# techshoww/RoMa

Measured on AMD Instinct MI355X. Metric: image-pairs/sec at 560->864, higher is better.
Workload: dtype fp16; 1 GPU; roma_outdoor 560->864 full coarse-to-fine symmetric match (BASELINE configs[1]; configs[2] = --pairs 8 --gpus 8); launch=eager launches, coarse_res=560, upsample_res=864, parallelism=single GPU

## Files before the change

include/roma_hip.h:

```cpp
#ifndef ROMA_HIP_H
#define ROMA_HIP_H

#include <stdint.h>

#ifdef __cplusplus
extern "C" {
#endif

#define ROMA_ABI_VERSION 5

enum { ROMA_F32 = 0, ROMA_F16 = 1, ROMA_BF16 = 2 };
enum { ROMA_NCHW = 0, ROMA_NHWC = 1 };
enum { ROMA_LC_AUTO = 0, ROMA_LC_TILE8X4 = 1, ROMA_LC_TILE8X8 = 2, ROMA_LC_ROWS8 = 3 };
enum { ROMA_E_ARG = -1, ROMA_E_DTYPE = -2, ROMA_E_SHAPE = -3, ROMA_E_ALIGN = -4, ROMA_E_UNSUPPORTED = -5 };

int roma_abi_version(void);
const char* roma_last_error(void);

int roma_local_corr(const void* f0, const void* f1, const float* flow, void* out,
                    int B, int C, int H, int W, int r, int dtype,
                    int layout, int f0_pitch, int f1_pitch, int out_layout, int out_pitch, int f1_batch_shift, int variant,
                    void* stream);

int roma_warp_bilinear(const void* src, const float* flow, void* dst,
                       int B, int C, int Hs, int Ws, int H, int W, int dtype,
                       int layout, int src_pitch, int dst_layout, int dst_pitch, int src_batch_shift, void* stream);

int roma_disp_emb(const float* flow, const float* weight, const float* bias, void* dst,
                  int B, int E, int H, int W, float gain, int dtype, int dst_layout, int dst_pitch, void* stream);

int roma_interp_bilinear(const float* x, float* y, int N, int Hi, int Wi, int Ho, int Wo, void* stream);

int roma_interp_bilinear_pair(const float* x0, float* y0, int N0, const float* x1, float* y1, int N1, int Hi, int Wi, int Ho, int Wo,
                              void* stream);

int roma_refiner_assemble(const void* src, const float* flow, const float* weight, const float* bias, void* buf, int B, int C, int E,
                          int D, int pitch, int Hs, int Ws, int H, int W, int src_pitch, int src_batch_shift, float gain, int dtype,
                          void* stream);

int roma_flow_update(float* flow, float* cert, const float* cert_in, const float* delta,
                     int B, int H, int W, float sx, float sy, void* stream);

int roma_cls_to_flow_refine(const void* logits, float* flow_out, float* cert_out,
                            int B, int C, int HW, long stride_b, long stride_c, long stride_p,
                            int dtype, void* stream);

int roma_cos_kernel(const void* x, const void* y, float* K, int B, int N, int M, int D, int dtype, int x_pitch, int y_pitch,
                    int y_batch_shift, float T, float eps, float diag_add, void* stream);

int roma_chol_diag_block(float* A, int lda, long strideA, float* W, int ldw, long strideW, int nb, int B, int* info,
                         int info_base, void* stream);

int roma_chol_step(float* A, int lda, long strideA, int n, int ncols, int j, int nb, const float* W, int ldw, long strideW, float* R,
                   int ldr, long strideR, float* Wn, int ldwn, long strideWn, int* info, int info_base, int B, void* stream);

int roma_chol_subst_step(int dir, const float* W, int ldw, long strideW, const float* R, long strideRb, long strideRs, int ldr, float* T,
                         long strideTb, long strideTs, int ldt, int t_in_panel, float* X, int ldx, long strideX, int n, int m, int nb,
                         int s, int B, void* stream);

int roma_attention_fwd(const void* q, const void* k, const void* v, void* o, int B, int H, int Nq, int Nk, int head_dim, long q_sb,
                       long q_sn, long q_sh, long k_sb, long k_sn, long k_sh, long v_sb, long v_sn, long v_sh, long o_sb, long o_sn,
                       long o_sh, float scale, int dtype, void* stream);

int roma_match_finalize(const float* flow, const float* cert, const float* cert16, float* warp, float* certainty,
                        int P, int H, int W, int H16, int W16, int symmetric, void* stream);

int roma_kde_density(const float* x, float* density, int N, int down, float std, int half_mode, void* stream);

int roma_race_keys(const float* p, const long* counter, float* keys, long N, float thresh, unsigned seed, unsigned stage,
                   void* stream);

long roma_race_select_workspace(int P, long N, int k);
int roma_race_select(const float* p, const long* counter, const long* seeds, int P, long N, int k, float thresh, unsigned stage,
                     long* sel_key, long* sel_idx, void* workspace, long workspace_bytes, void* stream);

int roma_kde_density_batch(const float* x, const long* index, float* density, int P, long N, int n, int down, float std,
                           int half_mode, void* stream);

int roma_nn_argmin(const float* q, const float* r, int* idx, int NQ, int NR, void* stream);

int roma_resample_u8(const void* in, void* out, int H, int W, int C, int out_size, int axis, const int* bounds,
                     const int* coef, int ksize, void* stream);
int roma_normalize_u8(const void* in, float* out, int H, int W, const float* mean3, const float* std3, void* stream);

int roma_bias_relu_nchw(void* x, const void* bias, int B, int C, int HW, int dtype, void* stream);

int roma_bias_relu_pool2_nchw(void* x, const void* bias, void* pooled, int B, int C, int H, int W, int dtype, void* stream);

int roma_bias_relu_nhwc(void* x, const void* bias, long npix, int C, int dtype, void* stream);
int roma_bias_relu_pool2_nhwc(void* x, const void* bias, void* pooled, int B, int C, int H, int W, int dtype, void* stream);

int roma_maxpool2_nhwc(const void* x, void* pooled, int B, int C, int H, int W, int dtype, void* stream);

int roma_conv3x3_bias_relu(const void* x, const void* w, const void* bias, void* y, int B, int Cin, int Cout, int H, int W, int dtype,
                           int x_pitch, int y_pitch, int instance, void* stream);
int roma_conv3x3_bias_relu_instances(int index, char* name, int cap);

int roma_dwconv5x5_bn_relu(const void* x, const float* w, const float* scale, const float* shift, void* y,
                           int B, int C, int H, int W, int dtype, int x_pitch, int y_pitch, void* stream);

int roma_refiner_block(const void* x, const void* w25, const float* scale, const float* shift, const void* wt,
                       const float* bias, void* y, int B, int C, int H, int W, int kpad, int dtype, int x_pitch, int y_pitch,
                       void* stream);

int roma_refiner_wide_pack(const void* wt, void* wp, int D);
int roma_refiner_wide_taps(const void* w25, void* w25p, int D);
int roma_refiner_block_wide(const void* x, const void* w25p, const float* scale, const float* shift, const void* wp,
                            const float* bias, void* y, int B, int H, int W, int D, int x_pitch, int y_pitch, int dtype,
                            void* stream);

int roma_pointwise_mfma(const void* x, const void* wt, const float* bias, void* y, long M, int C, int kpad, int dtype,
                        int x_pitch, int y_pitch, void* stream);

int roma_refiner_block_mid(const void* x, const float* w25, const float* scale, const float* shift, const void* wt,
                           const float* bias, void* y, int B, int C, int H, int W, int dtype, int x_pitch, int y_pitch,
                           void* stream);

int roma_refiner_head(const void* x, const float* wo, const float* bo, float* flow, const float* cert_in, float* cert_out,
                      float* delta_out, int B, int H, int W, int C, int pitch, int dtype, float sx, float sy, void* stream);

int roma_pointwise_small(const void* x, const float* wt, const float* bias, void* y, long M, int C, int dtype,
                         int x_pitch, int y_pitch, void* stream);

int roma_project_skinny(const void* x, const void* wt, const float* bias, void* y, long M, int K, int N, int dtype, int x_pitch,
                        int y_pitch, void* stream);

int roma_add_layernorm(void* x, int x_dtype, long x_stride, const void* y, int y_dtype, long y_stride, const float* ls,
                       const float* gamma, const float* beta, void* out, int out_dtype, long out_stride, long rows, int C,
                       float eps, void* stream);

int roma_tiny_corr_posembed(const float* f0, const float* f1, float* out, int B, int C,
// ... 114 lines not shown
```

roma_amd/_lib.py:

```python
from __future__ import annotations

import ctypes
import os
from ctypes import c_char_p, c_float, c_int, c_long, c_void_p

_HERE = os.path.dirname(os.path.abspath(__file__))
LIB_PATH = os.path.join(_HERE, "csrc", "libroma_hip.so")

ROMA_F32, ROMA_F16, ROMA_BF16 = 0, 1, 2
ROMA_NCHW, ROMA_NHWC = 0, 1
LC_VARIANTS = {"auto": 0, "tile8x4": 1, "tile8x8": 2, "rows8": 3}
ABI_VERSION = 5
SCORE_MSAC, SCORE_MAGSAC = 0, 1
ROMA_E_ARG, ROMA_E_DTYPE, ROMA_E_SHAPE, ROMA_E_ALIGN, ROMA_E_UNSUPPORTED = -1, -2, -3, -4, -5

SIGNATURES = {
    "roma_abi_version": [],
    "roma_last_error": [],
    "roma_local_corr": [c_void_p, c_void_p, c_void_p, c_void_p, c_int, c_int, c_int, c_int, c_int, c_int,
                        c_int, c_int, c_int, c_int, c_int, c_int, c_int, c_void_p],
    "roma_warp_bilinear": [c_void_p, c_void_p, c_void_p, c_int, c_int, c_int, c_int, c_int, c_int, c_int,
                           c_int, c_int, c_int, c_int, c_int, c_void_p],
    "roma_disp_emb": [c_void_p, c_void_p, c_void_p, c_void_p, c_int, c_int, c_int, c_int, c_float, c_int, c_int, c_int, c_void_p],
    "roma_interp_bilinear": [c_void_p, c_void_p, c_int, c_int, c_int, c_int, c_int, c_void_p],
    "roma_interp_bilinear_pair": [c_void_p, c_void_p, c_int, c_void_p, c_void_p, c_int, c_int, c_int, c_int, c_int, c_void_p],
    "roma_refiner_assemble": [c_void_p, c_void_p, c_void_p, c_void_p, c_void_p, c_int, c_int, c_int, c_int, c_int, c_int, c_int, c_int,
                              c_int, c_int, c_int, c_float, c_int, c_void_p],
    "roma_project_skinny": [c_void_p, c_void_p, c_void_p, c_void_p, c_long, c_int, c_int, c_int, c_int, c_int, c_void_p],
    "roma_flow_update": [c_void_p, c_void_p, c_void_p, c_void_p, c_int, c_int, c_int, c_float, c_float, c_void_p],
    "roma_cls_to_flow_refine": [c_void_p, c_void_p, c_void_p, c_int, c_int, c_int, c_long, c_long, c_long, c_int, c_void_p],
    "roma_cos_kernel": [c_void_p, c_void_p, c_void_p, c_int, c_int, c_int, c_int, c_int, c_int, c_int, c_int, c_float, c_float,
                        c_float, c_void_p],
    "roma_add_layernorm": [c_void_p, c_int, c_long, c_void_p, c_int, c_long, c_void_p, c_void_p, c_void_p, c_void_p, c_int, c_long,
                           c_long, c_int, c_float, c_void_p],
    "roma_attention_fwd": [c_void_p, c_void_p, c_void_p, c_void_p, c_int, c_int, c_int, c_int, c_int] + [c_long] * 12 + [c_float, c_int, c_void_p],
    "roma_chol_diag_block": [c_void_p, c_int, c_long, c_void_p, c_int, c_long, c_int, c_int, c_void_p, c_int, c_void_p],
    "roma_chol_step": [c_void_p, c_int, c_long, c_int, c_int, c_int, c_int, c_void_p, c_int, c_long, c_void_p, c_int, c_long,
                       c_void_p, c_int, c_long, c_void_p, c_int, c_int, c_void_p],
    "roma_chol_subst_step": [c_int, c_void_p, c_int, c_long, c_void_p, c_long, c_long, c_int, c_void_p, c_long, c_long, c_int, c_int,
                             c_void_p, c_int, c_long, c_int, c_int, c_int, c_int, c_int, c_void_p],
    "roma_match_finalize": [c_void_p, c_void_p, c_void_p, c_void_p, c_void_p, c_int, c_int, c_int, c_int, c_int, c_int, c_void_p],
    "roma_kde_density": [c_void_p, c_void_p, c_int, c_int, c_float, c_int, c_void_p],
    "roma_nn_argmin": [c_void_p, c_void_p, c_void_p, c_int, c_int, c_void_p],
    "roma_race_keys": [c_void_p, c_void_p, c_void_p, c_long, c_float, ctypes.c_uint, ctypes.c_uint, c_void_p],
    "roma_race_select_workspace": [c_int, c_long, c_int],
    "roma_race_select": [c_void_p, c_void_p, c_void_p, c_int, c_long, c_int, c_float, ctypes.c_uint, c_void_p, c_void_p, c_void_p, c_long,
                         c_void_p],
    "roma_kde_density_batch": [c_void_p, c_void_p, c_void_p, c_int, c_long, c_int, c_int, c_float, c_int, c_void_p],
    "roma_dwconv5x5_bn_relu": [c_void_p, c_void_p, c_void_p, c_void_p, c_void_p, c_int, c_int, c_int, c_int, c_int, c_int, c_int, c_void_p],
    "roma_resample_u8": [c_void_p, c_void_p, c_int, c_int, c_int, c_int, c_int, c_void_p, c_void_p, c_int, c_void_p],
    "roma_normalize_u8": [c_void_p, c_void_p, c_int, c_int, c_void_p, c_void_p, c_void_p],
    "roma_bias_relu_nchw": [c_void_p, c_void_p, c_int, c_int, c_int, c_int, c_void_p],
    "roma_bias_relu_pool2_nchw": [c_void_p, c_void_p, c_void_p, c_int, c_int, c_int, c_int, c_int, c_void_p],
    "roma_bias_relu_nhwc": [c_void_p, c_void_p, c_long, c_int, c_int, c_void_p],
    "roma_bias_relu_pool2_nhwc": [c_void_p, c_void_p, c_void_p, c_int, c_int, c_int, c_int, c_int, c_void_p],
    "roma_maxpool2_nhwc": [c_void_p, c_void_p, c_int, c_int, c_int, c_int, c_int, c_void_p],
    "roma_conv3x3_bias_relu": [c_void_p, c_void_p, c_void_p, c_void_p, c_int, c_int, c_int, c_int, c_int, c_int, c_int, c_int, c_int, c_void_p],
    "roma_conv3x3_bias_relu_instances": [c_int, c_char_p, c_int],
    "roma_pointwise_mfma": [c_void_p, c_void_p, c_void_p, c_void_p, c_long, c_int, c_int, c_int, c_int, c_int, c_void_p],
    "roma_refiner_block": [c_void_p, c_void_p, c_void_p, c_void_p, c_void_p, c_void_p, c_void_p, c_int, c_int, c_int, c_int, c_int, c_int,
                           c_int, c_int, c_void_p],
    "roma_refiner_block_mid": [c_void_p, c_void_p, c_void_p, c_void_p, c_void_p, c_void_p, c_void_p, c_int, c_int, c_int, c_int, c_int, c_int,
                               c_int, c_void_p],
    "roma_refiner_wide_pack": [c_void_p, c_void_p, c_int],
    "roma_refiner_wide_taps": [c_void_p, c_void_p, c_int],
    "roma_jpeg_info": [c_void_p, c_long, c_void_p],
    "roma_jpeg_entropy_decode": [c_void_p, c_long, c_void_p, c_void_p],
    "roma_jpeg_reconstruct": [c_void_p, c_void_p, c_void_p, c_void_p, c_void_p, c_void_p],
    "roma_refiner_block_wide": [c_void_p, c_void_p, c_void_p, c_void_p, c_void_p, c_void_p, c_void_p, c_int, c_int, c_int, c_int, c_int, c_int,
                                c_int, c_void_p],
    "roma_refiner_head": [c_void_p, c_void_p, c_void_p, c_void_p, c_void_p, c_void_p, c_void_p, c_int, c_int, c_int, c_int, c_int, c_int,
                          c_float, c_float, c_void_p],
    "roma_pointwise_small": [c_void_p, c_void_p, c_void_p, c_void_p, c_long, c_int, c_int, c_int, c_int, c_void_p],
    "roma_tiny_corr_posembed": [c_void_p, c_void_p, c_void_p, c_int, c_int, c_int, c_int, c_int, c_int, c_int, c_void_p],
    "roma_ransac_workspace": [c_int, c_int, c_int, c_int, c_void_p],
    "roma_ransac_hypotheses": [c_int, c_void_p, c_void_p, c_int, c_int, c_int, c_float, ctypes.c_uint, c_int, c_void_p, c_long, c_void_p],
    "roma_ransac_select": [c_int, c_void_p, c_void_p, c_int, c_int, c_int, c_float, c_int, c_void_p, c_long, c_void_p, c_void_p,
                           c_void_p],
    "roma_ransac_hypotheses_ex": [c_int, c_void_p, c_void_p, c_int, c_int, c_int, c_float, c_int, ctypes.c_uint, c_int, c_void_p, c_long,
                                  c_void_p],
    "roma_ransac_select_ex": [c_int, c_void_p, c_void_p, c_int, c_int, c_int, c_float, c_int, c_int, c_void_p, c_long, c_void_p, c_void_p,
                              c_void_p],
    "roma_magsac_table": [c_void_p, c_void_p],
    "roma_essential_workspace": [c_int, c_int, c_int, c_void_p],
    "roma_essential_hypotheses": [c_void_p, c_void_p, c_void_p, c_void_p, c_int, c_int, c_int, c_float, ctypes.c_uint, c_int, c_void_p,
                                  c_long, c_void_p],
    "roma_essential_select": [c_void_p, c_void_p, c_void_p, c_void_p, c_int, c_int, c_int, c_float, c_int, c_void_p, c_long, c_void_p,
                              c_void_p, c_void_p],
    "roma_essential_hypotheses_ex": [c_void_p, c_void_p, c_void_p, c_void_p, c_int, c_int, c_int, c_float, c_int, ctypes.c_uint, c_int,
                                     c_void_p, c_long, c_void_p],
    "roma_essential_select_ex": [c_void_p, c_void_p, c_void_p, c_void_p, c_int, c_int, c_int, c_float, c_int, c_int, c_void_p, c_long,
                                 c_void_p, c_void_p, c_void_p],
    "roma_recover_pose": [c_void_p, c_void_p, c_void_p, c_void_p, c_void_p, c_void_p, c_int, c_int, c_void_p, c_void_p, c_void_p,
                          c_void_p, c_void_p],
    "roma_refine_pose": [c_void_p, c_void_p, c_void_p, c_void_p, c_void_p, c_void_p, c_void_p, c_int, c_int, ctypes.c_double, c_int,
                         c_void_p, c_void_p, c_void_p, c_void_p, c_void_p, c_void_p, c_void_p],
    "roma_refine_fundamental": [c_void_p, c_void_p, c_void_p, c_void_p, c_int, c_int, ctypes.c_double, c_int, c_void_p, c_void_p, c_void_p,
                                c_void_p, c_void_p, c_void_p],
    "roma_refine_homography": [c_void_p, c_void_p, c_void_p, c_void_p, c_int, c_int, ctypes.c_double, c_int, c_void_p, c_void_p, c_void_p,
                               c_void_p, c_void_p, c_void_p],
    "roma_triangulate": [c_void_p, c_void_p, c_void_p, c_void_p, c_void_p, c_void_p, c_void_p, c_int, c_int, c_int, c_float, c_float,
                         c_void_p, c_void_p, c_void_p, c_void_p, c_void_p, c_void_p, c_void_p],
    "roma_triangulate_nview": [c_void_p, c_void_p, c_void_p, c_long, c_void_p, c_void_p, c_void_p, c_int, c_int, c_int, c_long, c_long,
                               c_float, c_int, c_int, c_int, c_float, c_float, c_void_p, c_void_p, c_void_p, c_void_p, c_void_p, c_void_p,
                               c_void_p],
    "roma_tracks_workspace": [c_int, c_void_p, c_int, c_void_p],
    "roma_build_tracks": [c_void_p, c_void_p, c_void_p, c_void_p, c_void_p, c_int, c_int, c_int, c_int, c_float, c_int, c_int, c_void_p,
                          c_void_p, c_void_p, c_void_p, c_void_p, c_void_p, c_void_p, c_long, c_void_p],
    "roma_warp_kpts": [c_void_p, c_int, c_void_p, c_void_p, c_void_p, c_void_p, c_void_p, c_int, c_int, c_int, c_int, c_int, c_int, c_int,
                       ctypes.c_double, c_void_p, c_void_p, c_void_p, c_void_p],
    "roma_dense_match_metrics": [c_void_p, c_long, c_void_p, c_void_p, c_void_p, c_void_p, c_void_p, c_int, c_int, c_int, c_int, c_int, c_int,
                                 c_int, c_int, ctypes.c_double, c_void_p, c_long, c_void_p, c_void_p, c_void_p, c_void_p, c_void_p],
    "roma_absolute_pose_workspace": [c_int, c_int, c_int, c_void_p],
    "roma_absolute_pose_hypotheses": [c_void_p, c_void_p, c_void_p, c_int, c_int, c_int, c_float, c_int, ctypes.c_uint, c_int, c_void_p,
                                      c_long, c_void_p],
# ... 63 lines not shown
```

roma_amd/csrc/cos_kernel.hip:

```cpp
#include "common.h"

namespace roma {
namespace {

typedef float f32x16 __attribute__((ext_vector_type(16)));
constexpr int BT = 64, KT = 16, LD = KT + 1;

template <typename T> __device__ __forceinline__ float4_t ld4(const T* p) {
  if constexpr (sizeof(T) == 4) {
    return *reinterpret_cast<const float4_t*>(p);
  } else {
    typedef T v4 __attribute__((ext_vector_type(4)));
    const v4 h = *reinterpret_cast<const v4*>(p);
    return float4_t{(float)h[0], (float)h[1], (float)h[2], (float)h[3]};
  }
}

template <typename T>
__global__ __launch_bounds__(256) void cos_kernel_mfma(const T* __restrict__ x, const T* __restrict__ y, float* __restrict__ K,
                                                       int N, int M, int D, int x_pitch, int y_pitch, int y_shift, float invT,
                                                       float eps, float diag_add) {
  __shared__ float sA[BT * LD], sB[BT * LD];
  __shared__ double sN[2 * BT];
  const int tid = threadIdx.x, lane = tid & 63, wave = tid >> 6;
  const int wr = wave >> 1, wc = wave & 1;
  const int b = blockIdx.z, n0 = blockIdx.y * BT, m0 = blockIdx.x * BT;
  const T* xb = x + (size_t)b * N * x_pitch;
  const T* yb = y + (size_t)((b + y_shift) % (int)gridDim.z) * M * y_pitch;
  f32x16 acc;
  double accd[16];
#pragma unroll
  for (int i = 0; i < 16; ++i) { acc[i] = 0.f; accd[i] = 0.0; }
  double nrm = 0.0;
  const int lr = tid >> 2, lc = (tid & 3) * 4;
  for (int k0 = 0; k0 < D; k0 += KT) {
    float4_t va{0, 0, 0, 0}, vb{0, 0, 0, 0};
    if (n0 + lr < N) va = ld4<T>(xb + (size_t)(n0 + lr) * x_pitch + k0 + lc);
    if (m0 + lr < M) vb = ld4<T>(yb + (size_t)(m0 + lr) * y_pitch + k0 + lc);
    __syncthreads();
#pragma unroll
    for (int i = 0; i < 4; ++i) {
      sA[lr * LD + lc + i] = va[i];
      sB[lr * LD + lc + i] = vb[i];
    }
    __syncthreads();
    if (tid < 2 * BT) {
      const float* r = (tid < BT ? sA : sB) + (tid & (BT - 1)) * LD;
#pragma unroll
      for (int i = 0; i < KT; ++i) nrm = __builtin_fma((double)r[i], (double)r[i], nrm);
    }
    const float* pa = sA + (wr * 32 + (lane & 31)) * LD + (lane >> 5);
    const float* pb = sB + (wc * 32 + (lane & 31)) * LD + (lane >> 5);
#pragma unroll
    for (int kk = 0; kk < KT; kk += 2) acc = __builtin_amdgcn_mfma_f32_32x32x2f32(pa[kk], pb[kk], acc, 0, 0, 0);
    if (((k0 / KT) & 3) == 3 || k0 + KT >= D) {
#pragma unroll
      for (int i = 0; i < 16; ++i) { accd[i] += (double)acc[i]; acc[i] = 0.f; }
    }
  }
  if (tid < 2 * BT) sN[tid] = sqrt(nrm);
  __syncthreads();
  const int col = lane & 31;
  const int m = m0 + wc * 32 + col;
  const double ny = sN[BT + wc * 32 + col];
#pragma unroll
  for (int r = 0; r < 16; ++r) {
    const int row = (r & 3) + 8 * (r >> 2) + 4 * (lane >> 5);
    const int n = n0 + wr * 32 + row;
    if (n < N && m < M) {
      const double c = accd[r] / (sN[wr * 32 + row] * ny + (double)eps);
      float v = (float)exp((c - 1.0) * (double)invT);
      if (n == m) v += diag_add;
      K[((size_t)b * N + n) * M + m] = v;
    }
  }
}

}
}

using namespace roma;

extern "C" int roma_cos_kernel(const void* x, const void* y, float* K, int B, int N, int M, int D, int dtype, int x_pitch,
                               int y_pitch, int y_batch_shift, float T, float eps, float diag_add, void* stream) {
  ROMA_REQUIRE(x && y && K, ROMA_E_ARG, "roma_cos_kernel: null pointer");
  ROMA_REQUIRE(B > 0 && N > 0 && M > 0 && D > 0, ROMA_E_SHAPE, "roma_cos_kernel: bad shape");
  ROMA_REQUIRE(D % KT == 0, ROMA_E_SHAPE, "roma_cos_kernel: D=%d must be a multiple of %d", D, KT);
  ROMA_REQUIRE(x_pitch >= D && y_pitch >= D, ROMA_E_SHAPE, "roma_cos_kernel: row pitch smaller than D");
  ROMA_REQUIRE(dtype >= ROMA_F32 && dtype <= ROMA_BF16, ROMA_E_DTYPE, "roma_cos_kernel: unknown dtype %d", dtype);
  const int e16 = dtype == ROMA_F32 ? 4 : 8;
  ROMA_REQUIRE(aligned16(x) && aligned16(y) && x_pitch % e16 == 0 && y_pitch % e16 == 0, ROMA_E_ALIGN,
               "roma_cos_kernel: x and y must be 16-byte aligned with row pitches that keep every row 16-byte aligned");
  ROMA_REQUIRE(y_batch_shift >= 0 && y_batch_shift < B, ROMA_E_ARG, "roma_cos_kernel: y_batch_shift %d outside [0, B)", y_batch_shift);
  ROMA_REQUIRE(T > 0.f, ROMA_E_ARG, "roma_cos_kernel: temperature must be positive");
  dim3 grid((M + BT - 1) / BT, (N + BT - 1) / BT, B);
  hipStream_t s = static_cast<hipStream_t>(stream);
#define ROMA_COS(TT)                                                                                                         \
  hipLaunchKernelGGL((cos_kernel_mfma<TT>), grid, dim3(256), 0, s, (const TT*)x, (const TT*)y, K, N, M, D, x_pitch, y_pitch, \
                     y_batch_shift, 1.f / T, eps, diag_add)
  if (dtype == ROMA_F32) ROMA_COS(float); else if (dtype == ROMA_F16) ROMA_COS(half_t); else ROMA_COS(bf16_t);
#undef ROMA_COS
  ROMA_CHECK_LAUNCH();
}
```

roma_amd/matcher.py:

```python
from __future__ import annotations

import math
import os
from collections import namedtuple
from typing import Dict, Optional
from warnings import warn

import numpy as np
import torch
import torch.nn as nn
import torch.nn.functional as F

from . import ops
from .transformer import Block, TransformerDecoder

IMAGENET_MEAN = (0.485, 0.456, 0.406)
IMAGENET_STD = (0.229, 0.224, 0.225)


def pixel_grid(b, h, w, device):
    ys = torch.linspace(-1 + 1 / h, 1 - 1 / h, h, device=device)
    xs = torch.linspace(-1 + 1 / w, 1 - 1 / w, w, device=device)
    return torch.stack((xs[None, :].expand(h, w), ys[:, None].expand(h, w)), dim=0)[None].expand(b, 2, h, w).contiguous()

# ... 168 lines not shown
                if impl == "split_mfma":
                    cur = ops.pointwise_mfma(rows, blk.wt_out_in, blk.bias, Dp)
                elif impl == "split_small":
                    cur = ops.pointwise_small(rows, blk.wt_in_out, blk.bias)
                else:
                    cur = torch.addmm(blk.bias, rows, blk.wt_in_out)
                cur = cur.view(B, h, w, Dp)
        return cur, P

    @torch.no_grad()
    def forward(self, x, y, flow, scale_factor=1, logits=None, dtype=None):
        flow = flow.float().contiguous()
        cur, P = self._body(x, y, flow, scale_factor, dtype or self.amp_dtype)
        B, h, w, Dp = cur.shape
        out = torch.addmm(P.bo, cur.reshape(B * h * w, Dp).float(), P.wo)
        out = out.view(B, h, w, self.out_dim).permute(0, 3, 1, 2).contiguous()
        return out[:, :-1], out[:, -1:]

    @torch.no_grad()
    def forward_update(self, x, y, flow, certainty, scale_factor, sx, sy, dtype=None, buf=None, batch_shift=0):
        cur, P = self._body(x, y, flow, scale_factor, dtype or self.amp_dtype, buf=buf, batch_shift=batch_shift)
        return ops.refiner_head(cur, P.wo, P.bo, flow, certainty, sx, sy)


class CosKernel(nn.Module):
    def __init__(self, T=0.2, learn_temperature=False):
        super().__init__()
        self.T = T

    def __call__(self, x, y, eps=1e-6):
        return ops.cos_kernel(x, y, T=self.T, eps=eps)


class GP(nn.Module):

    def __init__(self, gp_dim=512, T=0.2, sigma_noise=0.1, kernel=None, **_):
        super().__init__()
        self.K = CosKernel(T=T)
        self.sigma_noise = sigma_noise
        self.pos_conv = nn.Conv2d(2, gp_dim, 1, 1)
        self.dim = gp_dim
        self._basis = {}

    def basis(self, b, h, w, device):
        key = (h, w, device, _params_version(self.pos_conv))
        f = self._basis.get(key)
        if f is None:
            g = pixel_grid(1, h, w, device)
            f = torch.cos(8 * math.pi * F.conv2d(g, self.pos_conv.weight.float(), self.pos_conv.bias.float()))
            f = f.flatten(2).transpose(1, 2).contiguous()
            self._basis = {key: f}
        return f.expand(b, -1, -1)

    @torch.no_grad()
    def forward(self, x, y, **kwargs):
        b, c, h1, w1 = x.shape
        _, _, h2, w2 = y.shape
        xs = x.float().flatten(2).transpose(1, 2).contiguous()
        ys = y.float().flatten(2).transpose(1, 2).contiguous()
        K_yy = ops.cos_kernel(ys, ys, T=self.K.T, diag_add=self.sigma_noise)
        K_xy = ops.cos_kernel(xs, ys, T=self.K.T)
        mu = self.posterior_product(K_xy, ops.spd_solve(K_yy, self.basis(1, h2, w2, x.device)))
        return mu.transpose(1, 2).reshape(b, self.dim, h1, w1)

    def posterior_rows(self, xs, ys, h2, w2, fp64=False, batch_shift=0, out=None, check="now"):
        B, n = xs.shape[0], xs.shape[1]
        s = batch_shift % B
        basis = self.basis(1, h2, w2, xs.device)
        if fp64:
            a = xs.double()
            c = (a.roll(-s, 0) if s else a) if ys is None else ys.double()

            def cosk(u, v):
                g = torch.einsum("bnd,bmd->bnm", u, v) / (u.norm(dim=-1)[..., None] * v.norm(dim=-1)[:, None] + 1e-6)
                return ((g - 1.0) / self.K.T).exp()

            Kyy = cosk(c, c) + self.sigma_noise * torch.eye(c.shape[1], device=c.device, dtype=torch.float64)
            Z = torch.cholesky_solve(basis.double().expand(B, -1, -1), torch.linalg.cholesky(Kyy))
            mu = (cosk(a, c) @ Z).float()
            if out is not None:
                out.copy_(mu)
                return out
            return mu
        if ys is None:
            K_self = ops.cos_kernel(xs, xs, T=self.K.T, diag_add=self.sigma_noise)
            K_xy = ops.cos_kernel(xs, xs, T=self.K.T, batch_shift=s)
            Z = ops.spd_solve(K_self, basis, check=check)
            if s:
                assert 2 * s == B, "only the half swap of forward_symmetric"
                Z = torch.cat((Z[s:], Z[:s]), dim=0)
        else:
            K_yy = ops.cos_kernel(ys, ys, T=self.K.T, diag_add=self.sigma_noise)
            K_xy = ops.cos_kernel(xs, ys, T=self.K.T)
            Z = ops.spd_solve(K_yy, basis, check=check)
        return self.posterior_product(K_xy, Z, out)

    @staticmethod
    def posterior_product(K_xy, Z, out=None):
        mu = torch.bmm(K_xy.double(), Z.double())
        if out is None:
            return mu.float()
        out.copy_(mu)
        return out


class Decoder(nn.Module):
    def __init__(self, embedding_decoder, gps, proj, conv_refiner, detach=True, scales=("16", "8", "4", "2", "1"),
                 amp_dtype=torch.float16, **_):
        super().__init__()
        self.embedding_decoder, self.gps, self.proj, self.conv_refiner = embedding_decoder, gps, proj, conv_refiner
        self.scales = list(scales)
        self.refine_init = 4
        self.amp_dtype = amp_dtype
        self.gp_precision = "fp32"
        self.record = None
        self.flow_override = None
        self._proj = None

    def _embedding_decoder_for(self, dtype):
        if dtype == torch.float32:
            return self.embedding_decoder
        key = (dtype, _params_version(self.embedding_decoder))
        hit = self.__dict__.get("_embed_cast")
        if hit is None or hit[0] != key:
            import copy
            with torch.inference_mode(False), torch.no_grad():
                cp = copy.deepcopy(self.embedding_decoder).eval()
                for m in cp.modules():
                    if isinstance(m, nn.Linear):
                        m.to(dtype)
                hit = (key, cp)
            self.__dict__["_embed_cast"] = hit
        return hit[1]

    def get_placeholder_flow(self, b, h, w, device):
        return pixel_grid(b, h, w, device)

    def folded_proj(self, dtype):
        key = (dtype, _params_version(self.proj))
        if self._proj is not None and self._proj[0] == key:
            return self._proj[1]
        out = {}
        for s, seq in self.proj.items():
            conv, bn = seq[0], seq[1]
            g = bn.weight.float() / torch.sqrt(bn.running_var.float() + bn.eps)
            wt = (conv.weight.float().reshape(conv.out_channels, -1) * g[:, None]).t().contiguous().to(dtype)
            b = ((conv.bias.float() - bn.running_mean.float()) * g + bn.bias.float()).to(dtype)
            out[s] = (wt, b)
            if wt.shape[1] < 16:
                out[s + "/16"] = (F.pad(wt, (0, 16 - wt.shape[1])).contiguous(), F.pad(b, (0, 16 - b.shape[0])).contiguous())
            if project_impl(dtype, True, *wt.shape, 8) == "skinny":
                out[s + "/skinny"] = ops.project_skinny_pack(wt, b)
        self._proj = (key, out)
        return out

    def project(self, s, f, dtype, out=None):
        proj = self.folded_proj(dtype)
        wt, b = proj[s]
        B, C, h, w = f.shape
        f = f.to(dtype)
        n = wt.shape[1]
        dense_nhwc = f.stride() == (h * w * C, 1, w * C, C) and f.data_ptr() % 16 == 0
        if out is None:
            pitch = (n + 15) // 16 * 16 if project_impl(dtype, dense_nhwc, C, n, 8) == "skinny" else n
            out = torch.empty((B, h, w, pitch), dtype=dtype, device=f.device)[..., :n]
        out_rows = out.stride() == (h * w * out.stride(2), w * out.stride(2), out.stride(2), 1) and out.data_ptr() % 16 == 0
        if project_impl(dtype, dense_nhwc and out_rows, C, n, out.stride(2)) == "skinny":
            ops.project_skinny(f.permute(0, 2, 3, 1).reshape(B * h * w, C), *proj[s + "/skinny"], n,
                               out.as_strided((B * h * w, n), (out.stride(2), 1)))
            return out.permute(0, 3, 1, 2)
        tgt = out
        if n < 16 and out.stride(2) >= 16 and out.storage_offset() == 0:
            tgt = out.as_strided((B, h, w, 16), out.stride())
# ... 348 lines not shown
```

roma_amd/ops.py:

```python
from __future__ import annotations

import math
from typing import Optional

import torch

from . import _lib
from ._lib import ROMA_BF16, ROMA_F16, ROMA_F32, ROMA_NCHW, ROMA_NHWC, check

_DT = {torch.float32: ROMA_F32, torch.float16: ROMA_F16, torch.bfloat16: ROMA_BF16}


class KernelTimer:

    def __init__(self):
        self.enabled = False
        self.bracket_overhead_s = 0.0
        self.records = []

    def start(self):
        self.records.clear()
        torch.cuda.synchronize()
        pairs = []
        for _ in range(32):
# ... 174 lines not shown
    ya = torch.empty((B, Ca, Ho, Wo), dtype=torch.float32, device=a.device)
    yb = torch.empty((Bb, Cb, Ho, Wo), dtype=torch.float32, device=a.device)
    check(_lib.load().roma_interp_bilinear_pair(_p(a), _p(ya), B * Ca, _p(b), _p(yb), Bb * Cb, Hi, Wi, Ho, Wo, _stream()),
          "roma_interp_bilinear_pair")
    return ya, yb


def refiner_assemble(buf, src, flow, weight, bias, gain, C, D, batch_shift=0):
    _need_gpu(buf, src, flow, weight, bias)
    B, H, W, Dp = buf.shape
    E = weight.shape[0]
    ls, ps, s = feat_layout(src)
    if ls != ROMA_NHWC or s is not src or src.dtype != buf.dtype or not buf.is_contiguous():
        raise ValueError("refiner_assemble: buf must be contiguous (B,h,w,Dp), src channels-last and of buf's dtype")
    if tuple(flow.shape) != (B, 2, H, W) or src.shape[0] != B or src.shape[1] != C:
        raise ValueError(f"refiner_assemble: flow {tuple(flow.shape)} / src {tuple(src.shape)} do not match buf {tuple(buf.shape)}, C = {C}")
    flow = flow.float().contiguous()
    w = weight.reshape(E, 2).float().contiguous()
    bvec = bias.float().contiguous()
    check(_lib.load().roma_refiner_assemble(_p(src), _p(flow), _p(w), _p(bvec), _p(buf), B, C, E, D, Dp, src.shape[2], src.shape[3], H, W,
                                            ps, int(batch_shift) % B, float(gain), _dt(buf), _stream()), "roma_refiner_assemble")
    return buf


def flow_update(flow, certainty, delta, sx, sy):
    _need_gpu(flow, certainty, delta)
    B, _, H, W = flow.shape
    assert flow.dtype == torch.float32 and flow.is_contiguous() and delta.dtype == torch.float32 and delta.is_contiguous()
    cert_in = None if certainty is None else certainty.float().contiguous()
    cert = torch.empty((B, 1, H, W), dtype=torch.float32, device=flow.device)
    check(_lib.load().roma_flow_update(_p(flow), _p(cert), _p(cert_in), _p(delta), B, H, W, float(sx), float(sy), _stream()),
          "roma_flow_update")
    return flow, cert


def cls_to_flow_refine(cls):
    _need_gpu(cls)
    B, C, H, W = cls.shape
    sb, sc, sh, sw = cls.stride()
    if sh != W * sw:
        cls = cls.contiguous()
        sb, sc, sh, sw = cls.stride()
    flow = torch.empty((B, 2, H, W), dtype=torch.float32, device=cls.device)
    check(_lib.load().roma_cls_to_flow_refine(_p(cls), _p(flow), None, B, C, H * W, sb, sc, sw, _dt(cls), _stream()),
          "roma_cls_to_flow_refine")
    return flow.permute(0, 2, 3, 1)


def cls_rows_to_flow(rows, B, H, W):
    _need_gpu(rows)
    assert rows.dim() == 3 and rows.shape[0] == B and rows.shape[1] == H * W and rows.stride(2) == 1
    C = rows.shape[2] - 1
    flow = torch.empty((B, 2, H, W), dtype=torch.float32, device=rows.device)
    cert = torch.empty((B, 1, H, W), dtype=torch.float32, device=rows.device)
    check(_lib.load().roma_cls_to_flow_refine(_p(rows), _p(flow), _p(cert), B, C, H * W, rows.stride(0), 1, rows.stride(1),
                                              _dt(rows), _stream()), "roma_cls_to_flow_refine")
    return flow, cert


def _rows(t):
    B, N, D = t.shape
    es = t.element_size()
    if t.stride(2) == 1 and t.stride(0) == N * t.stride(1) and t.stride(1) >= D and (t.stride(1) * es) % 16 == 0 \
            and t.data_ptr() % 16 == 0 and t.dtype in _DT:
        return t, t.stride(1)
    t = (t if t.dtype in _DT else t.float()).contiguous()
    return t, D


def cos_kernel(x, y, T=0.2, eps=1e-6, diag_add=0.0, batch_shift=0):
    _need_gpu(x, y)
    if x.dtype != y.dtype:
        x, y = x.float(), y.float()
    x, xp = _rows(x)
    y, yp = _rows(y)
    B, N, D = x.shape
    M = y.shape[1]
    K = torch.empty((B, N, M), dtype=torch.float32, device=x.device)
    check(_lib.load().roma_cos_kernel(_p(x), _p(y), _p(K), B, N, M, D, _dt(x), xp, yp, int(batch_shift) % B, float(T), float(eps),
                                      float(diag_add), _stream()), "roma_cos_kernel")
    return K


class _PendingSpdCheck:

    def __init__(self, info):
        self.host = torch.empty(info.shape, dtype=info.dtype, pin_memory=True)
        self.host.copy_(info, non_blocking=True)
        self.event = torch.cuda.Event()
        self.event.record()

    def result(self):
        self.event.synchronize()
        return self.host.tolist()


_PENDING = []


def _raise_if_not_spd(bad):
    if any(bad):
        b = next(i for i, v in enumerate(bad) if v)
        raise _lib.RomaHipError(f"spd_solve: matrix {b} of the batch is not positive definite (block step {(bad[b] - 1) // 64}, pivot "
                                f"{(bad[b] - 1) % 64} is <= 0 or NaN) — non-finite or degenerate features?  The reference's "
                                f"torch.linalg.inv raises here too (matcher.py:261).")


_DEFER_DEPTH = [0]


def deferring():
    return _DEFER_DEPTH[0] > 0


class deferred_spd_checks:

    def __enter__(self):
        _DEFER_DEPTH[0] += 1
        return self

    def __exit__(self, et, ev, tb):
        _DEFER_DEPTH[0] -= 1
        if _DEFER_DEPTH[0] > 0:
            return False
        todo, _PENDING[:] = list(_PENDING), []
        if et is None and not torch.cuda.is_current_stream_capturing():
            for chk in todo:
                _raise_if_not_spd(chk.result())
        return False


def raise_pending():
    if torch.cuda.is_current_stream_capturing():
        return
    todo, _PENDING[:] = list(_PENDING), []
    for chk in todo:
        _raise_if_not_spd(chk.result())


def spd_solve(K, F, check="now", refine=0):
    _need_gpu(K, F)
    assert K.dtype == torch.float32 and F.dtype == torch.float32
    tun = torch.cuda.tunable.is_enabled()
    if tun:
        torch.cuda.tunable.enable(False)
    try:
        X, info = _spd_solve(K, F, refine)
    finally:
        if tun:
            torch.cuda.tunable.enable(True)
    if check == "now":
        _raise_if_not_spd(info.tolist())
    elif check == "defer":
        _PENDING.append(_PendingSpdCheck(info))
    return X


def _spd_solve(K, F, refine=0):
    nb = 64
    B, n, _ = K.shape
    m = F.shape[2]
    lib = _lib.load()
    A = torch.cat((K, F.expand(B, -1, -1)), dim=2)
    steps = [(j, min(j + nb, n)) for j in range(0, n, nb)]
    W = torch.empty((B, len(steps), nb, nb), dtype=torch.float32, device=K.device)
    info = torch.zeros((B,), dtype=torch.int32, device=K.device)
    Rall = torch.empty((B, len(steps), nb, n + m), dtype=torch.float32, device=K.device)
    check(lib.roma_chol_diag_block(A.data_ptr(), A.stride(1), A.stride(0), W.data_ptr(), nb, W.stride(0), steps[0][1], B,
                                   info.data_ptr(), 0, _stream()), "roma_chol_diag_block")
    for s, (j, e) in enumerate(steps):
        last = s + 1 == len(steps)
        check(lib.roma_chol_step(A.data_ptr(), A.stride(1), A.stride(0), n, n + m, j, e - j, W[:, s].data_ptr(), nb, W.stride(0),
                                 Rall[:, s].data_ptr(), n + m, Rall.stride(0), None if last else W[:, s + 1].data_ptr(), nb, W.stride(0),
                                 info.data_ptr(), nb * (s + 1), B, _stream()), "roma_chol_step")
    X = torch.empty((B, n, m), dtype=torch.float32, device=K.device)
    S = len(steps)

    def subst(direction, T, sTb, sTs, ldt, in_panel, out):
        for s in (range(S - 1, -1, -1) if direction < 0 else range(S)):
            check(lib.roma_chol_subst_step(direction, W[:, s].data_ptr(), nb, W.stride(0), Rall.data_ptr(), Rall.stride(0), Rall.stride(1),
                                           n + m, T.data_ptr(), sTb, sTs, ldt, in_panel, out.data_ptr(), m, out.stride(0), n, m, nb, s, B,
                                           _stream()), "roma_chol_subst_step")

    subst(-1, Rall, Rall.stride(0), Rall.stride(1), n + m, 1, X)
    for _ in range(int(refine)):
        g = (F.double() - torch.bmm(K.double(), X.double())).float().contiguous()
        y = torch.empty_like(g)
        subst(+1, g, g.stride(0), nb * m, m, 0, y)
        d = torch.empty_like(g)
        subst(-1, y, y.stride(0), nb * m, m, 0, d)
        X = X + d
    return X, info


def match_finalize(flow, certainty, cert16, symmetric=True):
    _need_gpu(flow, certainty, cert16)
    B, _, H, W = flow.shape
    P = B // 2 if symmetric else B
    flow = flow.float().contiguous()
    certainty = certainty.float().contiguous()
    H16 = W16 = 0
    if cert16 is not None:
        cert16 = cert16.float().contiguous()
        H16, W16 = cert16.shape[-2:]
    WW = 2 * W if symmetric else W
    warp = torch.empty((P, H, WW, 4), dtype=torch.float32, device=flow.device)
    cert = torch.empty((P, H, WW), dtype=torch.float32, device=flow.device)
    check(_lib.load().roma_match_finalize(_p(flow), _p(certainty), _p(cert16), _p(warp), _p(cert), P, H, W, H16, W16,
                                          1 if symmetric else 0, _stream()), "roma_match_finalize")
    return warp, cert


def kde(x, std=0.1, half=True, down=None):
    _need_gpu(x)
    if x.dim() != 2 or x.shape[1] != 4:
        raise ValueError("kde expects (N,4) matches")
    xs = (x.half() if half else x).float().contiguous()
    N = xs.shape[0]
    dens = torch.empty((N,), dtype=torch.float32, device=x.device)
    check(_lib.load().roma_kde_density(_p(xs), _p(dens), N, int(down or 1), float(std), 1 if half else 0, _stream()), "roma_kde_density")
    return dens.half() if half else dens


def race_keys(p, thresh=-1.0, seed=0, counter=None, stage=0):
    _need_gpu(p, counter)
    p = p.reshape(-1).float().contiguous()
    if counter is not None:
        counter = counter.reshape(-1).long().contiguous()
        assert counter.numel() == p.numel()
    keys = torch.empty_like(p)
    check(_lib.load().roma_race_keys(_p(p), _p(counter), _p(keys), p.numel(), float(thresh), int(seed) & 0xFFFFFFFF,
                                     int(stage) & 0xFFFFFFFF, _stream()), "roma_race_keys")
    return keys


def seed_tensor(seeds, P, device):
    if seeds is None:
        seeds = torch.randint(0, 2 ** 31 - 1, (P,))
    if not torch.is_tensor(seeds):
        seeds = torch.tensor([int(s) & 0xFFFFFFFF for s in seeds], dtype=torch.int64)
    seeds = seeds.reshape(-1).to(torch.int64)
    if seeds.numel() != P:
        raise ValueError(f"{P} pairs need {P} seeds, got {seeds.numel()}")
    if not seeds.is_cuda:
        seeds = seeds.pin_memory().to(device, non_blocking=True)
    return seeds.contiguous()


def race_select(p, k, thresh=-1.0, seeds=None, counter=None, stage=0):
    _need_gpu(p, counter)
    if p.dim() != 2:
        raise ValueError("race_select expects (P,N) weights")
    if seeds is None:
        raise ValueError("race_select needs P seeds")
    p = p.float().contiguous()
    P, N = p.shape
    k = int(k)
    seeds = seed_tensor(seeds, P, p.device)
# ... 349 lines not shown
```

Before: 61.94 image-pairs/s.

## Fuse symmetric self and cross cosine kernels into one launch with mirrored tiles

Adds a paired cosine-kernel launch that computes only upper-triangular tiles of each self kernel and mirrors them through a shared-memory transpose. For the half-swapped cross kernel it computes one tile for both batch halves and writes it to both. The self kernel is written straight into the augmented Cholesky buffer, which removes the separate concatenation copy. This cuts launches, roughly halves the dot-product work, and drops one large copy, in exchange for more complex indexing and transposed stores.

```diff
diff --git a/include/roma_hip.h b/include/roma_hip.h
--- a/include/roma_hip.h
+++ b/include/roma_hip.h
@@ -47,6 +47,9 @@
 
 int roma_cos_kernel(const void* x, const void* y, float* K, int B, int N, int M, int D, int dtype, int x_pitch, int y_pitch,
                     int y_batch_shift, float T, float eps, float diag_add, void* stream);
+
+int roma_cos_kernel_pair(const void* x, float* K_self, int ldk, long self_batch_stride, float* K_xy, int B, int N, int D, int dtype,
+                         int x_pitch, int shift, float T, float eps, float diag_add, void* stream);
 
 int roma_chol_diag_block(float* A, int lda, long strideA, float* W, int ldw, long strideW, int nb, int B, int* info,
                          int info_base, void* stream);
diff --git a/roma_amd/_lib.py b/roma_amd/_lib.py
--- a/roma_amd/_lib.py
+++ b/roma_amd/_lib.py
@@ -31,6 +31,8 @@
     "roma_cls_to_flow_refine": [c_void_p, c_void_p, c_void_p, c_int, c_int, c_int, c_long, c_long, c_long, c_int, c_void_p],
     "roma_cos_kernel": [c_void_p, c_void_p, c_void_p, c_int, c_int, c_int, c_int, c_int, c_int, c_int, c_int, c_float, c_float,
                         c_float, c_void_p],
+    "roma_cos_kernel_pair": [c_void_p, c_void_p, c_int, c_long, c_void_p, c_int, c_int, c_int, c_int, c_int, c_int, c_float, c_float,
+                             c_float, c_void_p],
     "roma_add_layernorm": [c_void_p, c_int, c_long, c_void_p, c_int, c_long, c_void_p, c_void_p, c_void_p, c_void_p, c_int, c_long,
                            c_long, c_int, c_float, c_void_p],
     "roma_attention_fwd": [c_void_p, c_void_p, c_void_p, c_void_p, c_int, c_int, c_int, c_int, c_int] + [c_long] * 12 + [c_float, c_int, c_void_p],
diff --git a/roma_amd/csrc/cos_kernel.hip b/roma_amd/csrc/cos_kernel.hip
--- a/roma_amd/csrc/cos_kernel.hip
+++ b/roma_amd/csrc/cos_kernel.hip
@@ -17,18 +17,11 @@
 }
 
 template <typename T>
-__global__ __launch_bounds__(256) void cos_kernel_mfma(const T* __restrict__ x, const T* __restrict__ y, float* __restrict__ K,
-                                                       int N, int M, int D, int x_pitch, int y_pitch, int y_shift, float invT,
-                                                       float eps, float diag_add) {
-  __shared__ float sA[BT * LD], sB[BT * LD];
-  __shared__ double sN[2 * BT];
+__device__ __forceinline__ void cos_tile_sums(const T* __restrict__ xb, const T* __restrict__ yb, int n0, int m0, int N, int M, int D,
+                                              int x_pitch, int y_pitch, float* sA, float* sB, double* sN, double (&accd)[16]) {
   const int tid = threadIdx.x, lane = tid & 63, wave = tid >> 6;
   const int wr = wave >> 1, wc = wave & 1;
-  const int b = blockIdx.z, n0 = blockIdx.y * BT, m0 = blockIdx.x * BT;
-  const T* xb = x + (size_t)b * N * x_pitch;
-  const T* yb = y + (size_t)((b + y_shift) % (int)gridDim.z) * M * y_pitch;
   f32x16 acc;
-  double accd[16];
 #pragma unroll
   for (int i = 0; i < 16; ++i) { acc[i] = 0.f; accd[i] = 0.0; }
   double nrm = 0.0;
@@ -60,6 +53,26 @@
   }
   if (tid < 2 * BT) sN[tid] = sqrt(nrm);
   __syncthreads();
+}
+
+__device__ __forceinline__ float cos_entry(double dot, double nx, double ny, float eps, float invT) {
+  const double c = dot / (nx * ny + (double)eps);
+  return (float)exp((c - 1.0) * (double)invT);
+}
+
+template <typename T>
+__global__ __launch_bounds__(256) void cos_kernel_mfma(const T* __restrict__ x, const T* __restrict__ y, float* __restrict__ K,
+                                                       int N, int M, int D, int x_pitch, int y_pitch, int y_shift, float invT,
+                                                       float eps, float diag_add) {
+  __shared__ float sA[BT * LD], sB[BT * LD];
+  __shared__ double sN[2 * BT];
+  const int lane = threadIdx.x & 63, wave = threadIdx.x >> 6;
+  const int wr = wave >> 1, wc = wave & 1;
+  const int b = blockIdx.z, n0 = blockIdx.y * BT, m0 = blockIdx.x * BT;
+  const T* xb = x + (size_t)b * N * x_pitch;
+  const T* yb = y + (size_t)((b + y_shift) % (int)gridDim.z) * M * y_pitch;
+  double accd[16];
+  cos_tile_sums<T>(xb, yb, n0, m0, N, M, D, x_pitch, y_pitch, sA, sB, sN, accd);
   const int col = lane & 31;
   const int m = m0 + wc * 32 + col;
   const double ny = sN[BT + wc * 32 + col];
@@ -68,10 +81,76 @@
     const int row = (r & 3) + 8 * (r >> 2) + 4 * (lane >> 5);
     const int n = n0 + wr * 32 + row;
     if (n < N && m < M) {
-      const double c = accd[r] / (sN[wr * 32 + row] * ny + (double)eps);
-      float v = (float)exp((c - 1.0) * (double)invT);
+      float v = cos_entry(accd[r], sN[wr * 32 + row], ny, eps, invT);
       if (n == m) v += diag_add;
       K[((size_t)b * N + n) * M + m] = v;
+    }
+  }
+}
+
+constexpr int TP = BT + 1;
+
+template <typename T>
+__global__ __launch_bounds__(256) void cos_pair_kernel(const T* __restrict__ x, float* __restrict__ K_self, int ldk,
+                                                       long self_batch_stride, float* __restrict__ K_xy, int B, int N, int D,
+                                                       int x_pitch, int shift, float invT, float eps, float diag_add) {
+  __shared__ float sT[BT * TP];
+  __shared__ double sN[2 * BT];
+  static_assert(2 * BT * LD <= BT * TP, "the staging tiles must fit in the transpose buffer");
+  const int lane = threadIdx.x & 63, wave = threadIdx.x >> 6;
+  const int wr = wave >> 1, wc = wave & 1;
+  const int nt = (N + BT - 1) / BT, tri = nt * (nt + 1) / 2;
+  int id = blockIdx.x, bx, by, ti, tj;
+  float *direct, *mirror;
+  long pitch;
+  bool self = id < B * tri;
+  if (self) {
+    bx = by = id / tri;
+    const int t = id - bx * tri;
+    tj = (int)((sqrtf(8.f * (float)t + 1.f) - 1.f) * 0.5f);
+    while (tj * (tj + 1) / 2 > t) --tj;
+    while ((tj + 1) * (tj + 2) / 2 <= t) ++tj;
+    ti = t - tj * (tj + 1) / 2;
+    pitch = ldk;
+    direct = K_self + (size_t)bx * self_batch_stride;
+    mirror = ti == tj ? nullptr : direct;
+  } else {
+    id -= B * tri;
+    bx = id / (nt * nt);
+    by = bx + shift;
+    const int t = id - bx * nt * nt;
+    ti = t / nt;
+    tj = t - ti * nt;
+    pitch = N;
+    direct = K_xy + (size_t)bx * N * N;
+    mirror = K_xy + (size_t)by * N * N;
+  }
+  const int n0 = ti * BT, m0 = tj * BT;
+  double accd[16];
+  cos_tile_sums<T>(x + (size_t)bx * N * x_pitch, x + (size_t)by * N * x_pitch, n0, m0, N, N, D, x_pitch, x_pitch, sT, sT + BT * LD, sN,
+                   accd);
+  const int col = lane & 31;
+  const int m = m0 + wc * 32 + col;
+  const double ny = sN[BT + wc * 32 + col];
+#pragma unroll
+  for (int r = 0; r < 16; ++r) {
+    const int row = (r & 3) + 8 * (r >> 2) + 4 * (lane >> 5);
+    const int n = n0 + wr * 32 + row;
+    float v = cos_entry(accd[r], sN[wr * 32 + row], ny, eps, invT);
+    if (self && n == m) v += diag_add;
+    sT[(wr * 32 + row) * TP + wc * 32 + col] = v;
+  }
+  __syncthreads();
+#pragma unroll 4
+  for (int r = 0; r < 16; ++r) {
+    const int row = wave * 16 + r;
+    if (n0 + row < N && m0 + lane < N) direct[(size_t)(n0 + row) * pitch + m0 + lane] = sT[row * TP + lane];
+  }
+  if (mirror != nullptr) {
+#pragma unroll 4
+    for (int r = 0; r < 16; ++r) {
+      const int row = wave * 16 + r;
+      if (m0 + row < N && n0 + lane < N) mirror[(size_t)(m0 + row) * pitch + n0 + lane] = sT[lane * TP + row];
     }
   }
 }
@@ -102,3 +181,28 @@
 #undef ROMA_COS
   ROMA_CHECK_LAUNCH();
 }
+
+extern "C" int roma_cos_kernel_pair(const void* x, float* K_self, int ldk, long self_batch_stride, float* K_xy, int B, int N, int D,
+                                    int dtype, int x_pitch, int shift, float T, float eps, float diag_add, void* stream) {
+  ROMA_REQUIRE(x && K_self && K_xy, ROMA_E_ARG, "roma_cos_kernel_pair: null pointer");
+  ROMA_REQUIRE(B > 0 && N > 0 && D > 0, ROMA_E_SHAPE, "roma_cos_kernel_pair: bad shape");
+  ROMA_REQUIRE(D % KT == 0, ROMA_E_SHAPE, "roma_cos_kernel_pair: D=%d must be a multiple of %d", D, KT);
+  ROMA_REQUIRE(x_pitch >= D, ROMA_E_SHAPE, "roma_cos_kernel_pair: row pitch smaller than D");
+  ROMA_REQUIRE(dtype >= ROMA_F32 && dtype <= ROMA_BF16, ROMA_E_DTYPE, "roma_cos_kernel_pair: unknown dtype %d", dtype);
+  const int e16 = dtype == ROMA_F32 ? 4 : 8;
+  ROMA_REQUIRE(aligned16(x) && x_pitch % e16 == 0, ROMA_E_ALIGN,
+               "roma_cos_kernel_pair: x must be 16-byte aligned with a row pitch that keeps every row 16-byte aligned");
+  ROMA_REQUIRE(shift > 0 && 2 * shift == B, ROMA_E_ARG, "roma_cos_kernel_pair: shift %d is not half of B=%d", shift, B);
+  ROMA_REQUIRE(ldk >= N, ROMA_E_SHAPE, "roma_cos_kernel_pair: ldk=%d smaller than N=%d", ldk, N);
+  ROMA_REQUIRE(self_batch_stride >= (long)(N - 1) * ldk + N, ROMA_E_SHAPE, "roma_cos_kernel_pair: the items of K_self overlap");
+  ROMA_REQUIRE(T > 0.f, ROMA_E_ARG, "roma_cos_kernel_pair: temperature must be positive");
+  const long nt = (N + BT - 1) / BT, tiles = B * (nt * (nt + 1) / 2) + shift * nt * nt;
+  ROMA_REQUIRE(tiles <= 0x7fffffffL, ROMA_E_SHAPE, "roma_cos_kernel_pair: %ld tiles do not fit one grid", tiles);
+  hipStream_t s = static_cast<hipStream_t>(stream);
+#define ROMA_COS(TT)                                                                                                           \
+  hipLaunchKernelGGL((cos_pair_kernel<TT>), dim3((unsigned)tiles), dim3(256), 0, s, (const TT*)x, K_self, ldk, self_batch_stride, K_xy, \
+                     B, N, D, x_pitch, shift, 1.f / T, eps, diag_add)
+  if (dtype == ROMA_F32) ROMA_COS(float); else if (dtype == ROMA_F16) ROMA_COS(half_t); else ROMA_COS(bf16_t);
+#undef ROMA_COS
+  ROMA_CHECK_LAUNCH();
+}
diff --git a/roma_amd/matcher.py b/roma_amd/matcher.py
--- a/roma_amd/matcher.py
+++ b/roma_amd/matcher.py
@@ -274,13 +274,16 @@
                 out.copy_(mu)
                 return out
             return mu
-        if ys is None:
+        if ys is None and s and 2 * s == B:
+            A = ops.spd_augmented(basis, B)
+            _, K_xy = ops.cos_kernel_pair(xs, T=self.K.T, diag_add=self.sigma_noise, batch_shift=s, self_out=A[:, :, :n])
+            Z = ops.spd_solve_augmented(A, check=check)
+            Z = torch.cat((Z[s:], Z[:s]), dim=0)
+        elif ys is None:
+            assert s == 0, "only the half swap of forward_symmetric"
             K_self = ops.cos_kernel(xs, xs, T=self.K.T, diag_add=self.sigma_noise)
-            K_xy = ops.cos_kernel(xs, xs, T=self.K.T, batch_shift=s)
+            K_xy = ops.cos_kernel(xs, xs, T=self.K.T)
             Z = ops.spd_solve(K_self, basis, check=check)
-            if s:
-                assert 2 * s == B, "only the half swap of forward_symmetric"
-                Z = torch.cat((Z[s:], Z[:s]), dim=0)
         else:
             K_yy = ops.cos_kernel(ys, ys, T=self.K.T, diag_add=self.sigma_noise)
             K_xy = ops.cos_kernel(xs, ys, T=self.K.T)
diff --git a/roma_amd/ops.py b/roma_amd/ops.py
--- a/roma_amd/ops.py
+++ b/roma_amd/ops.py
@@ -280,6 +280,24 @@
     return K
 
 
+def cos_kernel_pair(x, T=0.2, eps=1e-6, diag_add=0.0, batch_shift=0, self_out=None):
+    _need_gpu(x)
+    x, xp = _rows(x)
+    B, N, D = x.shape
+    s = int(batch_shift) % B
+    if 2 * s != B:
+        raise ValueError(f"cos_kernel_pair: batch_shift {batch_shift} is not half of the batch of {B}")
+    if self_out is None:
+        self_out = torch.empty((B, N, N), dtype=torch.float32, device=x.device)
+    if self_out.dtype != torch.float32 or self_out.device != x.device or self_out.dim() != 3 or self_out.shape[0] != B \
+            or self_out.shape[1] != N or self_out.shape[2] < N or self_out.stride(2) != 1:
+        raise ValueError(f"cos_kernel_pair: self_out must be a ({B},{N},>={N}) fp32 view with unit column stride on {x.device}")
+    K_xy = torch.empty((B, N, N), dtype=torch.float32, device=x.device)
+    check(_lib.load().roma_cos_kernel_pair(_p(x), _p(self_out), self_out.stride(1), self_out.stride(0), _p(K_xy), B, N, D, _dt(x), xp, s,
+                                           float(T), float(eps), float(diag_add), _stream()), "roma_cos_kernel_pair")
+    return self_out[:, :, :N], K_xy
+
+
 class _PendingSpdCheck:
 
     def __init__(self, info):
@@ -339,11 +357,30 @@
 def spd_solve(K, F, check="now", refine=0):
     _need_gpu(K, F)
     assert K.dtype == torch.float32 and F.dtype == torch.float32
+    return _spd_solve_checked(K, F, check, refine)
+
+
+def spd_augmented(F, B):
+    _need_gpu(F)
+    assert F.dtype == torch.float32
+    n, m = F.shape[-2:]
+    A = torch.empty((B, n, n + m), dtype=torch.float32, device=F.device)
+    A[:, :, n:] = F
+    return A
+
+
+def spd_solve_augmented(A, check="now"):
+    _need_gpu(A)
+    assert A.dtype == torch.float32 and A.dim() == 3 and A.is_contiguous() and A.shape[2] > A.shape[1]
+    return _spd_solve_checked(None, None, check, 0, A)
+
+
+def _spd_solve_checked(K, F, check, refine, A=None):
     tun = torch.cuda.tunable.is_enabled()
     if tun:
         torch.cuda.tunable.enable(False)
     try:
-        X, info = _spd_solve(K, F, refine)
+        X, info = _spd_solve(K, F, refine, A)
     finally:
         if tun:
             torch.cuda.tunable.enable(True)
@@ -354,16 +391,19 @@
     return X
 
 
-def _spd_solve(K, F, refine=0):
+def _spd_solve(K, F, refine=0, A=None):
     nb = 64
-    B, n, _ = K.shape
-    m = F.shape[2]
     lib = _lib.load()
-    A = torch.cat((K, F.expand(B, -1, -1)), dim=2)
+    if A is None:
+        A = torch.cat((K, F.expand(K.shape[0], -1, -1)), dim=2)
+    else:
+        assert not refine, "refinement needs K and F, which a caller-built A no longer holds after the factorisation"
+    B, n = A.shape[0], A.shape[1]
+    m = A.shape[2] - n
     steps = [(j, min(j + nb, n)) for j in range(0, n, nb)]
-    W = torch.empty((B, len(steps), nb, nb), dtype=torch.float32, device=K.device)
-    info = torch.zeros((B,), dtype=torch.int32, device=K.device)
-    Rall = torch.empty((B, len(steps), nb, n + m), dtype=torch.float32, device=K.device)
+    W = torch.empty((B, len(steps), nb, nb), dtype=torch.float32, device=A.device)
+    info = torch.zeros((B,), dtype=torch.int32, device=A.device)
+    Rall = torch.empty((B, len(steps), nb, n + m), dtype=torch.float32, device=A.device)
     check(lib.roma_chol_diag_block(A.data_ptr(), A.stride(1), A.stride(0), W.data_ptr(), nb, W.stride(0), steps[0][1], B,
                                    info.data_ptr(), 0, _stream()), "roma_chol_diag_block")
     for s, (j, e) in enumerate(steps):
@@ -371,7 +411,7 @@
         check(lib.roma_chol_step(A.data_ptr(), A.stride(1), A.stride(0), n, n + m, j, e - j, W[:, s].data_ptr(), nb, W.stride(0),
                                  Rall[:, s].data_ptr(), n + m, Rall.stride(0), None if last else W[:, s + 1].data_ptr(), nb, W.stride(0),
                                  info.data_ptr(), nb * (s + 1), B, _stream()), "roma_chol_step")
-    X = torch.empty((B, n, m), dtype=torch.float32, device=K.device)
+    X = torch.empty((B, n, m), dtype=torch.float32, device=A.device)
     S = len(steps)
 
     def subst(direction, T, sTb, sTs, ldt, in_panel, out):
```

Result: no change. 62.36 image-pairs/s, median of 6 (+0.7%).
